# Arash-san/YinYang-Game-AlphaZero

Measured on AMD Instinct MI355X. Metric: self-play positions/sec (+ MCTS node-expansions/sec) at 800 sims, 8x8 board, higher is better.
Workload: dtype f16x3; 1 GPU; 8x8 board, 800 sims/move, 4096 concurrent games per GPU, frozen random-init 128x10 net (seed 0), copied boards, reference_quirks=False, staggered start plies; tree_arithmetic=f32 PUCT + u64 bitboards, nn_dtype=f16x3, evaluation_reuse=False, parallelism=episode-sharded x1, lanes_per_gpu=2, hipgraph=True

## Files before the change

### yinyang-game-alphazero_amd/csrc/yy_common.h

```cpp
#pragma once
#include <hip/hip_runtime.h>
#include <stdio.h>

#include "../../include/yy_engine.h"

extern "C" int yy_tower_set_err(int code, const char *msg);

extern "C" __attribute__((visibility("hidden"))) int yy_mcts_step_noise(yy_mcts *ctx, const float *policy, const float *value, const double *noise, double eps,
                                  float *planes, uint8_t *needs_eval, yy_stream_t stream);

static inline int yy_hip_fail(const char *what, hipError_t e) {
    char msg[512];
    snprintf(msg, sizeof msg, "%s: %s", what, hipGetErrorString(e));
    return yy_tower_set_err(YY_E_HIP, msg);
}
#define HIP_TRY(x)                                        \
    do {                                                  \
        hipError_t e_ = (x);                              \
        if (e_ != hipSuccess) return yy_hip_fail(#x, e_); \
    } while (0)

__device__ __forceinline__ float relu_keep_nan(float v) { return __builtin_isnan(v) ? v : fmaxf(v, 0.0f); }

template <int N> __device__ __forceinline__ void wait_vmcnt() { asm volatile("s_waitcnt vmcnt(%0)" ::"n"(N) : "memory"); }
```

### yinyang-game-alphazero_amd/csrc/yy_engine.hip

```cpp
#include <hip/hip_runtime.h>
#include <math.h>
#include <stdio.h>
#include <string.h>

#include "../../include/yy_engine.h"
#include "yy_bitboard.h"
#include "yy_common.h"
#include "yy_tree.h"

#define YY_VERSION 109

static thread_local char g_err[512] = "";
static int set_err(int code, const char *fmt, const char *a = "", const char *b = "") {
    snprintf(g_err, sizeof g_err, fmt, a, b);
    return code;
}

extern "C" const char *yy_last_error(void) { return g_err; }
extern "C" int yy_tower_set_err(int code, const char *msg) { return set_err(code, "%s%s", msg); }
extern "C" int yy_version(void) { return YY_VERSION; }

static int check_geo(int G, int R, int C) {
    if (G <= 0 || R <= 0 || C <= 0) return set_err(YY_E_INVALID, "non-positive size%s%s");
    if (R > YY_MAX_DIM || C > YY_MAX_DIM || R * C > 64 * YY_MAX_NW)
// ... 624 lines not shown
            const int cell = j * 64 + lane;
            if ((mask.w[j] >> lane) & 1) {
                float p = prow[d.sym ? sym_cell(d.geo, s, cell) : cell];
                bad |= (p != p);
                if (mix) {
                    const float kp = __fmul_rn(keep, p);
                    p = (float)__dadd_rn((double)kp, __dmul_rn(eps, noise[(size_t)g * A + cell]));
                }
                edges[base + mbcnt(mask.w[j])] =
                    make_uint4(__float_as_uint(p), 0u, 0u, CHILD_NONE | ((uint32_t)cell << 24));
            }
            base += yy_popc64(mask.w[j]);
        }
        if (__ballot(bad)) return false;
        if (lane == 0) {
            nodes[node] = make_uint4((uint32_t)n_edges, node_pack(k, (hold && k == 0) ? NF_HASVALUE : 0u, lplayer), 0u,
                                     __float_as_uint(v));
            st->ctr[3] += (uint64_t)k;
        }
        n_edges += k;
    }
    if (lane == 0) {
        st->n_nodes = n_nodes;
        st->n_edges = n_edges;
    }
    return true;
}

__device__ __forceinline__ void backup_path(uint4 *edges, const int32_t *path, const int depth, const float v,
                                            const bool v_is_py, GameState *st) {
    const int lane = lane_id();
    for (int i = lane; i < depth; i += 64) {
        uint4 *e = edges + path[i];
        const int dist = depth - (i + 1);
        const float sv = (dist & 1) ? -v : v;
        uint4 r = *e;
        r.y = (uint32_t)((int)r.y + 1);
        r.z = __float_as_uint(__fadd_rn(__uint_as_float(r.z), sv));
        *e = r;
    }
    if (lane == 0) {
        const float sv = (depth & 1) ? -v : v;
        st->root_N += 1;
        if (st->root_w_is_py && v_is_py && depth == 0) {
            st->root_W_py += (double)((sv == 0.0001f) ? 0.0001 : (sv == -0.0001f ? -0.0001 : (double)sv));
        } else {
            const float base = st->root_w_is_py ? (float)st->root_W_py : st->root_W;
            st->root_W = __fadd_rn(base, sv);
            st->root_w_is_py = 0;
        }
    }
}

template <int NW> __global__ void __launch_bounds__(64) k_begin(MctsDev d, MultiDev m, int target, int kept_target,
                                                                const int32_t *budgets, int max_sims, const int8_t *boards,
                                                                const int8_t *players, const uint8_t *active,
                                                                float *planes) {
    const int g = blockIdx.x;
    const int K = m.K;
    GameState *st = d.state + g;
    LeafRec *rec = K > 1 ? m.leaves + (size_t)g * K : &st->leaf;
    const bool act = active ? (active[g] != 0) : true;
    BB<NW> black, white;
    board_to_bb<NW>(boards + (size_t)g * d.geo.A, d.geo.A, black, white);
    bool keep = false;
    if (rfl((int)st->kept)) {
        const uint64_t *nb = d.nboard + (size_t)g * d.node_cap * 2 * NW;
        const BB<NW> kb = bb_uniform_load<NW>(nb), kw = bb_uniform_load<NW>(nb + NW);
        bool same = act && rfl((int)players[g]) == rfl((int)st->root_player);
#pragma unroll
        for (int i = 0; i < NW; i++) same = same && kb.w[i] == black.w[i] && kw.w[i] == white.w[i];
        keep = same;
    }
    if (keep) {
        if (lane_id() == 0) {
            st->kept = 0;
            st->root_kept = 1;
            st->active = 1;
            st->err = 0;
            st->budget = budgets ? min(max(budgets[g], 0), max_sims) : kept_target;
            rec->kind = K_ROOTKEPT;
            rec->node = 0;
            rec->path_len = 0;
            rec->dup = -1;
        }
    }
    root_setup<NW>(d, st, rec, g, black, white, rfl((int)players[g]), act, keep,
                   budgets ? min(max(budgets[g], 0), max_sims) : target, planes + (size_t)g * K * 5 * d.geo.A);
    if (K > 1 && lane_id() == 0) {
        m.mst[2 * g] = budgets ? min(max(budgets[g], 0), max_sims) : target;
        m.mst[2 * g + 1] = act ? 1 : 0;
    }
}

template <int NW>
__device__ __forceinline__ void do_select(const MctsDev &d, const int g, float *planes, uint8_t *needs_eval,
                                          const uint32_t stamp) {
    GameState *st = d.state + g;
    const int lane = lane_id();
    const int s_active = st->active, s_err = st->err, s_budget = st->budget;
    const int s_kept = st->root_kept;
    int s_carry = st->root_N;
    s_carry = rfl(s_carry);
    if ((rfl(s_active) == 0) | (rfl(s_err) != 0) | (s_carry >= rfl(s_budget))) {
        if (lane == 0) {
            st->leaf.kind = K_NONE;
            if (needs_eval) needs_eval[g] = 0;
        }
        return;
    }
    s_carry -= rfl(s_kept);
// ... 137 lines not shown
    }
    if (!any) return;
    const float keep = (float)(1.0 - eps);
    for (int j = lane; j < k; j += 64) {
        uint4 *e = edges + first + j;
        const float kp = __fmul_rn(keep, __uint_as_float(e->x));
        e->x = __float_as_uint((float)__dadd_rn((double)kp, __dmul_rn(eps, nrow[e->w >> 24])));
    }
}

template <int NW>
__device__ __forceinline__ void do_expand_backup(const MctsDev &d, const int g, const float *policy,
                                                 const float *value, const double *noise, const double eps,
                                                 const uint32_t stamp) {
    GameState *st = d.state + g;
    const int lane = lane_id();
    const int kind = rfl((int)st->leaf.kind);
    if (kind == K_NONE) return;
    const uint4 *nodes = d.nodes + (size_t)g * d.node_cap;
    uint4 *edges = d.edges + (size_t)g * d.edge_cap;
    if (kind == K_ROOTKEPT) {
        if (noise) noise_kept_root(d, g, nodes, edges, noise, eps);
        if (lane == 0) st->leaf.kind = K_NONE;
        return;
    }
    const int32_t *path = d.path + (size_t)g * d.path_cap;
    const int depth = rfl(st->leaf.path_len);
    const int node = rfl(st->leaf.node);
    float v;
    bool v_is_py = false;
    if (kind == K_TERMINAL) {
        v = rflf(__uint_as_float(nodes[node].z));
        v_is_py = true;
    } else if (kind == K_REUSE) {
        v = rflf(__uint_as_float(nodes[node].w));
    } else {
        const bool root = kind == K_ROOTINIT;
        const int src = (root || !(d.ec.meta || d.bk.meta || d.sh.meta)) ? SRC_NONE : rfl(st->leaf_src);
        const LeafEval ev = leaf_eval<NW>(d, g, src, policy, root ? nullptr : value);
        v = ev.v;
        const bool hold = d.reuse && !root;
        if (!expand_leaf<NW>(d, st, g, &st->leaf, path, ev.prow, v, hold, d.aliased != 0u, root ? noise : nullptr, eps)) {
            if (lane == 0) { st->err = st->err_ever = 1; st->leaf.kind = K_NONE; }
            return;
        }
        if (d.ec.meta && src == SRC_NONE && !root) cache_store<NW>(d, st, g, policy, v);
        if (d.sh.meta && src == SRC_NONE && !root) shared_store<NW>(d, st, g, policy, v, stamp);
    }
    if (lane == 0) st->leaf.kind = K_NONE;
    if (kind == K_ROOTINIT) return;
    backup_path(edges, path, depth, v, v_is_py, st);
}

template <int NW> __global__ void __launch_bounds__(64) k_mcts(MctsDev d, int do_backup, int do_sel,
                                                               const float *policy, const float *value,
                                                               const double *noise, double eps, float *planes,
                                                               uint8_t *needs_eval) {
    const int g = blockIdx.x;
    const uint32_t stamp = d.sh.meta ? rfl(*d.sh_stamp) : 0u;
    if (do_backup) do_expand_backup<NW>(d, g, policy, value, noise, eps, stamp);
    if (do_backup && do_sel) __syncthreads();
    if (do_sel) do_select<NW>(d, g, planes, needs_eval, stamp);
}

__global__ void k_stamp(uint32_t *stamp) {
    if (blockIdx.x != 0 || threadIdx.x != 0) return;
    *stamp = sh_next_stamp(*stamp);
}

template <int NW>
__device__ __forceinline__ void do_select_multi(const MctsDev &d, const MultiDev &m, const int g, float *planes,
                                                uint8_t *needs_eval) {
    GameState *st = d.state + g;
    const int lane = lane_id();
    const int K = m.K;
    int32_t *ms = m.mst + 2 * g;
    int keff = 0;
    if (rfl((int)st->active) && !rfl((int)st->err)) keff = min(K, max(0, rfl(ms[0]) - rfl(st->root_N)));
    const GeoBB<NW> gb = geo_bb<NW>(d.geo);
    const uint4 *nodes = d.nodes + (size_t)g * d.node_cap;
    const uint4 *edges = d.edges + (size_t)g * d.edge_cap;
    uint64_t c_levels = 0, c_scan = 0, c_evals = 0, c_term = 0;
    bool failed = false;
    for (int j = 0; j < keff; j++) {
        int32_t *path = d.path + ((size_t)g * K + j) * d.path_cap;
        int node = 0, depth = 0, parent = -1, action = -1, kind;
        uint64_t match = (1ull << j) - 1ull;
        for (;;) {
            const uint4 hdr = nodes[node];
            const uint32_t hy = rfl(hdr.y);
            const int k = node_k(hy), first = rfl((int)hdr.x);
            if (node_flags(hy) & NF_TERMINAL) { kind = K_TERMINAL; break; }
            if (k == 0) { kind = (node == 0) ? K_ROOTPASS : K_REEXPAND; break; }
            if (depth >= (int)d.path_cap) { kind = K_NONE; break; }
            const int vi = ((match >> lane) & 1) ? d.path[((size_t)g * K + lane) * d.path_cap + depth] - first : -1;
            int v[NW];
#pragma unroll
            for (int t = 0; t < NW; t++) v[t] = 0;
            for (uint64_t mm = match; mm; mm &= mm - 1ull) {
                const int c = __builtin_amdgcn_readlane(vi, (int)__ffsll((unsigned long long)mm) - 1);
#pragma unroll
                for (int t = 0; t < NW; t++) v[t] += (c == t * 64 + lane) ? 1 : 0;
            }
            uint4 e[NW];
            uint32_t part = 0;
#pragma unroll
            for (int t = 0; t < NW; t++) {
                const int jj = t * 64 + lane;
                e[t] = (jj < k) ? edges[first + jj] : make_uint4(0u, 0u, 0u, 0u);
                part += e[t].y + (uint32_t)v[t];
            }
            const int S = (int)wave_uadd(part);
            const float sq = d.sqrt_tab[min(S, d.sqrt_n - 1)];
            float q0 = 0.0f;
// ... 7 lines not shown
                    }
                }
                q0 = fpu_value(fp, depth == 0 ? d.fpu_root : d.fpu);
            }
            uint32_t bk = 0, bw = 0;
            int bi = BEST_NONE;
#pragma unroll
            for (int t = 0; t < NW; t++) {
                const int jj = t * 64 + lane;
                if (jj < k) {
                    const float W = __uint_as_float(e[t].z);
                    const float w = (v[t] > 0) ? __fsub_rn(W, (float)v[t]) : W;
                    const uint32_t key = child_key(d.cpuct, sq, __uint_as_float(e[t].x), (int)e[t].y + v[t], w, q0);
                    if (key > bk) { bk = key; bi = jj; bw = e[t].w; }
                }
            }
            const int best = best_child(bk, bi, k);
            if (best == BEST_NONE) { kind = K_NONE; break; }
            const uint32_t w = (uint32_t)__builtin_amdgcn_readlane((int)bw, best & 63);
            if (lane == 0) path[depth] = first + best;
            match = __ballot(vi == best);
            depth++;
            c_levels++;
            c_scan += (uint64_t)k;
            parent = node;
            action = (int)(w >> 24);
            const uint32_t child = w & CHILD_NONE;
            if (child == CHILD_NONE) { kind = K_EXPAND; node = -1; break; }
            node = (int)child;
        }
        if (kind == K_NONE) { failed = true; break; }
        const int dup = match ? (int)__ffsll((unsigned long long)match) - 1 : -1;
        const bool need = (kind == K_EXPAND || kind == K_REEXPAND || kind == K_ROOTPASS) && dup < 0;
        LeafRec *rec = m.leaves + (size_t)g * K + j;
        if (need) {
            BB<NW> black, white;
            const int lplayer = leaf_position<NW>(d, st, g, nodes, kind, parent, action, false, black, white);
            BB<NW> mask;
            bool term;
            float tv;
            leaf_rules<NW>(d.geo, gb, black, white, lplayer, mask, term, tv);
            write_eval_planes<NW>(planes + ((size_t)g * K + j) * 5 * d.geo.A, d.geo, d.sym, d.sym_seed, black, white);
            leaf_store<NW>(rec, black, white, mask, lplayer, term, tv);
        }
        if (lane == 0) {
            rec->kind = (uint8_t)kind;
            rec->node = node;
            rec->path_len = depth;
            rec->dup = dup;
            if (needs_eval) needs_eval[(size_t)g * K + j] = need;
        }
        c_evals += need ? 1 : 0;
        c_term += (kind == K_TERMINAL) ? 1 : 0;
        __syncthreads();
    }
    if (failed && lane == 0) st->err = st->err_ever = 1;
    if (needs_eval && lane < K && (failed || lane >= keff)) needs_eval[(size_t)g * K + lane] = 0;
    if (lane == 0) {
        ms[1] = failed ? 0 : keff;
        st->ctr[1] += c_levels;
        st->ctr[2] += c_scan;
        if (!failed) st->ctr[0] += c_evals;
        st->ctr[4] += c_term;
    }
}

template <int NW>
__device__ __forceinline__ void do_expand_backup_multi(const MctsDev &d, const MultiDev &m, const int g, const float *policy,
                                                       const float *value, const double *noise, const double eps) {
    GameState *st = d.state + g;
    const int lane = lane_id();
    const int K = m.K;
    int32_t *ms = m.mst + 2 * g;
    const int nl = rfl(ms[1]);
    if (nl == 0) return;
    const uint4 *nodes = d.nodes + (size_t)g * d.node_cap;
    uint4 *edges = d.edges + (size_t)g * d.edge_cap;
    for (int j = 0; j < nl; j++) {
        const LeafRec *rec = m.leaves + (size_t)g * K + j;
        const int kind = rfl((int)rec->kind);
        const int depth = rfl(rec->path_len);
        const int dup = rfl(rec->dup);
        const int32_t *path = d.path + ((size_t)g * K + j) * d.path_cap;
        const size_t row = (size_t)g * K + (dup >= 0 ? dup : j);
        float v;
        bool v_is_py = false;
        if (kind == K_TERMINAL) {
            v = rflf(__uint_as_float(nodes[rfl(rec->node)].z));
            v_is_py = true;
        } else if (dup >= 0) {
            v = rflf(value[row]);
        } else {
            v = (kind == K_ROOTINIT) ? 0.0f : rflf(value[row]);
            if (!expand_leaf<NW>(d, st, g, rec, path, policy + row * d.geo.A, v, false, false, noise, eps)) {
                if (lane == 0) { st->err = st->err_ever = 1; ms[1] = 0; }
                return;
            }
        }
        if (kind == K_ROOTINIT) break;
        backup_path(edges, path, depth, v, v_is_py, st);
        __syncthreads();
    }
    if (lane == 0) ms[1] = 0;
}

template <int NW> __global__ void __launch_bounds__(64) k_mcts_multi(MctsDev d, MultiDev m, int do_backup, int do_sel,
                                                                     const float *policy, const float *value,
                                                                     const double *noise, double eps, float *planes,
                                                                     uint8_t *needs_eval) {
    const int g = blockIdx.x;
    if (do_backup) do_expand_backup_multi<NW>(d, m, g, policy, value, noise, eps);
    if (do_backup && do_sel) __syncthreads();
    if (do_sel) do_select_multi<NW>(d, m, g, planes, needs_eval);
}

template <int NW> __global__ void __launch_bounds__(64) k_advance(MctsDev d, const int32_t *actions, int32_t *kept_visits,
                                                                  int32_t *remap_all) {
    __shared__ int32_t win[64];
    const int g = blockIdx.x, lane = lane_id();
    GameState *st = d.state + g;
    uint4 *nodes = d.nodes + (size_t)g * d.node_cap;
    uint4 *edges = d.edges + (size_t)g * d.edge_cap;
    uint64_t *nboard = d.nboard + (size_t)g * d.node_cap * 2 * NW;
    int32_t *remap = remap_all + (size_t)g * d.node_cap;
    const int n_nodes = rfl(st->n_nodes), n_edges = rfl(st->n_edges);
    const int a = rfl(actions[g]);
    const uint4 rhdr = nodes[0];
    const int rk = node_k(rfl(rhdr.y)), rfirst = rfl((int)rhdr.x);
    int child = -1, keptN = 0;
    float keptW = 0.0f;
    bool ok = rfl((int)st->active) != 0 && rfl((int)st->err) == 0 && a >= 0 && a < d.geo.A && n_nodes <= (int)d.node_cap &&
              rk > 0 && rfirst >= 0 && rfirst + rk <= n_edges && n_edges <= (int)d.edge_cap;
    if (ok) {
        ok = false;
        for (int j0 = 0; j0 < rk; j0 += 64) {
            const int j = j0 + lane;
            const uint4 e = (j < rk) ? edges[rfirst + j] : make_uint4(0u, 0u, 0u, 0xFF000000u | CHILD_NONE);
            const uint64_t hit = __ballot(j < rk && (int)(e.w >> 24) == a);
            if (hit) {
                const int l = (int)__ffsll((unsigned long long)hit) - 1;
                const uint32_t w = (uint32_t)__builtin_amdgcn_readlane((int)e.w, l);
                keptN = __builtin_amdgcn_readlane((int)e.y, l);
                keptW = __uint_as_float((uint32_t)__builtin_amdgcn_readlane((int)e.z, l));
                child = (int)(w & CHILD_NONE);
                ok = (w & CHILD_NONE) != CHILD_NONE && child > 0 && child < n_nodes;
                break;
            }
        }
    }
    uint32_t chy = 0;
    if (ok) {
        chy = rfl(nodes[child].y);
        ok = !(node_flags(chy) & NF_TERMINAL) && node_k(chy) > 0;
    }
    if (!ok) {
        if (lane == 0) {
            st->kept = 0;
            st->n_nodes = 1;
            st->n_edges = 0;
            st->root_N = 0;
            st->root_W = 0.0f;
            st->root_W_py = 0.0;
            st->root_w_is_py = 1;
            nodes[0] = make_uint4(0u, node_pack(0, 0, node_player(rfl(rhdr.y))), 0u, 0u);
            if (kept_visits) kept_visits[g] = 0;
// ... 20 lines not shown
            for (int j0 = 0; j0 < k; j0 += 64) {
                const int j = j0 + lane;
                if (j < k) {
                    const uint4 e = edges[first + j];
                    edges[ne + j] = e;
                    const int c = (int)(e.w & CHILD_NONE);
                    if ((e.w & CHILD_NONE) != CHILD_NONE && c > i && c < n_nodes) {
                        if (c < base + 64) win[c - base] = 0;
                        else remap[c] = 0;
                    }
                }
            }
            if (lane == 0) {
                nodes[rank] = make_uint4(k > 0 ? (uint32_t)ne : 0u, hy, (uint32_t)__builtin_amdgcn_readlane((int)hdr.z, t),
                                         (uint32_t)__builtin_amdgcn_readlane((int)hdr.w, t));
                remap[i] = rank;
            }
            if (rank != i && lane < 2 * NW) nboard[(size_t)rank * 2 * NW + lane] = nboard[(size_t)i * 2 * NW + lane];
            rank++;
            ne += k;
            __syncthreads();
        }
        if (bad) break;
    }
    __syncthreads();
    if (!bad)
        for (int e = lane; e < ne; e += 64) {
            const uint32_t w = edges[e].w;
            const uint32_t c = w & CHILD_NONE;
            if (c != CHILD_NONE) {
                const int nc = (c < (uint32_t)n_nodes) ? remap[c] : -1;
                edges[e].w = (w & 0xFF000000u) | (nc >= 0 ? (uint32_t)nc : CHILD_NONE);
            }
        }
    if (lane == 0) {
        if (bad) {
            st->err = st->err_ever = 1;
            st->kept = 0;
            if (kept_visits) kept_visits[g] = 0;
        } else {
            st->n_nodes = rank;
            st->n_edges = ne;
            st->root_N = keptN;
            st->root_W = keptW;
            st->root_W_py = 0.0;
            st->root_w_is_py = 0;
            st->root_player = (int8_t)node_player(chy);
            st->kept = 1;
            if (kept_visits) kept_visits[g] = keptN;
        }
    }
}

template <int NW> __global__ void __launch_bounds__(64) k_root_counts(MctsDev d, int32_t *counts, float *cw, float *cp) {
    const int g = blockIdx.x, A = d.geo.A;
    const uint4 hdr = d.nodes[(size_t)g * d.node_cap];
    const int k = node_k(rfl(hdr.y)), first = rfl((int)hdr.x);
    const bool act = rfl((int)d.state[g].active) != 0;
    for (int a = lane_id(); a < A; a += 64) {
        counts[(size_t)g * A + a] = 0;
        if (cw) cw[(size_t)g * A + a] = 0.0f;
        if (cp) cp[(size_t)g * A + a] = 0.0f;
    }
    __syncthreads();
    if (!act) return;
    const uint4 *edges = d.edges + (size_t)g * d.edge_cap;
    for (int j = lane_id(); j < k; j += 64) {
        const uint4 e = edges[first + j];
        const int a = (int)(e.w >> 24);
        counts[(size_t)g * A + a] = (int)e.y;
        if (cw) cw[(size_t)g * A + a] = __uint_as_float(e.z);
        if (cp) cp[(size_t)g * A + a] = __uint_as_float(e.x);
    }
}

template <int NW> __global__ void __launch_bounds__(64) k_root_policy(MctsDev d, int tzero, double *pi) {
    root_distribution<NW>(d, blockIdx.x, tzero, pi + (size_t)blockIdx.x * d.geo.A);
}

__global__ void k_root_stats(MctsDev d, int32_t *visits, double *wsum) {
    const int g = blockIdx.x * blockDim.x + threadIdx.x;
    if (g >= d.G) return;
    const GameState *st = d.state + g;
    if (visits) visits[g] = st->root_N;
    if (wsum) wsum[g] = st->root_w_is_py ? st->root_W_py : (double)st->root_W;
}

template <int NW> __global__ void __launch_bounds__(64) k_get_boards(MctsDev d, int8_t *boards) {
    const int g = blockIdx.x;
    const uint64_t *src = d.gboard + (size_t)g * 2 * NW;
    BB<NW> b = bb_uniform_load<NW>(src), w = bb_uniform_load<NW>(src + NW);
    bb_to_board<NW>(boards + (size_t)g * d.geo.A, d.geo.A, b, w);
}

__global__ void k_status(MctsDev d, uint64_t *out ) {
    uint64_t acc[9] = {0, 0, 0, 0, 0, 0, 0, 0, 0};
    for (int g = blockIdx.x * blockDim.x + threadIdx.x; g < d.G; g += gridDim.x * blockDim.x) {
        GameState *st = d.state + g;
        for (int i = 0; i < 8; i++) acc[i] += st->ctr[i];
        acc[8] += (st->err || st->err_ever) ? 1 : 0;
        st->err_ever = 0;
    }
    for (int i = 0; i < 9; i++)
        if (acc[i]) atomicAdd((unsigned long long *)&out[i], (unsigned long long)acc[i]);
}

__global__ void k_reset_counters(MctsDev d) {
    const int g = blockIdx.x * blockDim.x + threadIdx.x;
    if (g >= d.G) return;
    for (int i = 0; i < 8; i++) d.state[g].ctr[i] = 0;
    d.state[g].forced = 0;
    for (int i = 0; i < 4; i++) d.state[g].shc[i] = 0;
    if (g == 0 && d.sh_sweep) d.sh_sweep[SH_SW_EVICTED] = 0;
}

__global__ void k_forced_sum(MctsDev d, uint64_t *out) {
    uint64_t acc = 0;
    for (int g = blockIdx.x * blockDim.x + threadIdx.x; g < d.G; g += gridDim.x * blockDim.x) acc += d.state[g].forced;
    if (acc) atomicAdd((unsigned long long *)out, (unsigned long long)acc);
}

extern "C" int yy_mcts_create(const yy_mcts_config *cfg, yy_mcts **out) {
    if (!cfg || !out) return set_err(YY_E_INVALID, "null pointer%s%s");
    if (int e = check_geo(cfg->G, cfg->R, cfg->C)) return e;
    if (cfg->max_sims < 1) return set_err(YY_E_INVALID, "max_sims < 1%s%s");
    if ((cfg->flags & YY_FLAG_REUSE_PASS_VALUE) && (cfg->flags & YY_FLAG_ALIASED))
        return set_err(YY_E_INVALID, "YY_FLAG_REUSE_PASS_VALUE needs copied boards: with the aliased board a node's position changes between visits%s%s");
    if ((cfg->flags & YY_FLAG_EVAL_SYMMETRY) && (cfg->flags & YY_FLAG_ALIASED))
        return set_err(YY_E_UNSUPPORTED, "YY_FLAG_EVAL_SYMMETRY needs copied boards (YY_FLAG_ALIASED reproduces the reference, which has no such option)%s%s");
    if (cfg->flags & YY_FLAG_FORCED_PLAYOUTS) {
// ... 76 lines not shown
            *a.p = nullptr;
            yy_mcts_destroy(c);
            return set_err(YY_E_NOMEM, "hipMalloc failed: %s%s", hipGetErrorString(me), what);
        }
        c->bytes += a.n;
    }
    float *tab = new float[d.sqrt_n];
    for (int s = 0; s < d.sqrt_n; s++) tab[s] = (float)sqrt((double)s);
    hipError_t e = hipMemset(d.state, 0, G * sizeof(GameState));
    if (e == hipSuccess) e = hipMemset(d.nodes, 0, G * d.node_cap * sizeof(uint4));
    if (e == hipSuccess && d.ec.meta) e = hipMemset(d.ec.meta, 0, G * (size_t)ec_cap * sizeof(uint32_t));
    if (e == hipSuccess && m.mst) e = hipMemset(m.mst, 0, G * 2 * sizeof(int32_t));
    if (e == hipSuccess) e = hipMemcpy(d.sqrt_tab, tab, (size_t)d.sqrt_n * sizeof(float), hipMemcpyHostToDevice);
    if (e == hipSuccess) e = hipDeviceSynchronize();
    delete[] tab;
    if (e != hipSuccess) { yy_mcts_destroy(c); return set_err(YY_E_HIP, "arena initialisation: %s%s", hipGetErrorString(e)); }
    *out = c;
    return YY_OK;
}

extern "C" int yy_mcts_destroy(yy_mcts *c) {
    if (!c) return YY_OK;
    const MctsDev &d = c->dev;
    void *ps[] = {d.edges, d.nodes, d.nboard, d.gboard, d.path, d.state, d.sqrt_tab, c->scratch, d.ec.meta, d.ec.key, d.ec.val, d.ec.pol,
                  c->multi.leaves, c->multi.mst, c->remap};
    for (void *p : ps)
        if (p) (void)hipFree(p);
    delete c;
    return YY_OK;
}

extern "C" int yy_mcts_set_num_sims(yy_mcts *c, int32_t num_sims) {
    if (!c) return set_err(YY_E_INVALID, "null pointer%s%s");
    if (num_sims < 0 || num_sims > c->cfg.max_sims) return set_err(YY_E_INVALID, "num_sims outside 0 .. max_sims%s%s");
    c->target_sims = num_sims == 0 ? c->cfg.max_sims : num_sims;
    return YY_OK;
}

extern "C" int yy_mcts_set_sim_budgets(yy_mcts *c, const int32_t *budgets_dev) {
    if (!c) return set_err(YY_E_INVALID, "null pointer%s%s");
    c->budgets = budgets_dev;
    return YY_OK;
}

extern "C" int yy_mcts_memory_bytes(const yy_mcts *c, uint64_t *out) {
    if (!c || !out) return set_err(YY_E_INVALID, "null pointer%s%s");
    *out = c->bytes;
    return YY_OK;
}

extern "C" int yy_mcts_begin(yy_mcts *c, const int8_t *boards, const int8_t *players, const uint8_t *active,
                             float *planes, yy_stream_t s) {
    if (!c || !boards || !players || !planes) return set_err(YY_E_INVALID, "null pointer%s%s");
    DISPATCH_NW(c->dev.geo.NW, k_begin<NW><<<dim3(c->cfg.G), dim3(64), 0, (hipStream_t)s>>>(c->dev, c->multi,
                                                   c->multi.K > 1 ? c->target_sims : 0x7FFFFFFF, c->target_sims, c->budgets, c->cfg.max_sims,
                                                   boards, players, active, planes));
    HIP_TRY(hipGetLastError());
    c->pending = 2;
    return YY_OK;
}

extern "C" int yy_mcts_advance(yy_mcts *c, const int32_t *actions, int32_t *kept_visits, yy_stream_t s) {
    if (!c || !actions) return set_err(YY_E_INVALID, "null pointer%s%s");
    if (c->cfg.flags & YY_FLAG_ALIASED)
        return set_err(YY_E_UNSUPPORTED, "yy_mcts_advance needs copied boards: with the aliased board a node's position changes between visits%s%s");
    if (c->multi.K > 1) return set_err(YY_E_UNSUPPORTED, "yy_mcts_advance: leaves_per_step > 1 does not support tree reuse%s%s");
    if (c->pending != 0) return set_err(YY_E_STATE, "yy_mcts_advance with a select or a root expansion pending%s%s");
    if (!c->remap) {
        const size_t n = (size_t)c->cfg.G * c->dev.node_cap * sizeof(int32_t);
        const hipError_t me = hipMalloc((void **)&c->remap, n);
        if (me != hipSuccess) {
            (void)hipGetLastError();
            c->remap = nullptr;
            return set_err(YY_E_NOMEM, "hipMalloc failed: %s%s", hipGetErrorString(me), " (tree reuse remap array)");
        }
        c->bytes += n;
    }
    DISPATCH_NW(c->dev.geo.NW, k_advance<NW><<<dim3(c->cfg.G), dim3(64), 0, (hipStream_t)s>>>(c->dev, actions, kept_visits, c->remap));
    HIP_TRY(hipGetLastError());
    return YY_OK;
}

static int launch_mcts(yy_mcts *c, int backup, int sel, const float *policy, const float *value, const double *noise,
                       double eps, float *planes, uint8_t *needs_eval, yy_stream_t s) {
    if (c->dev.sh.meta) {
        hipLaunchKernelGGL(k_stamp, dim3(1), dim3(1), 0, (hipStream_t)s, c->dev.sh_stamp);
        HIP_TRY(hipGetLastError());
    }
    if (c->multi.K > 1) {
        DISPATCH_NW(c->dev.geo.NW, k_mcts_multi<NW><<<dim3(c->cfg.G), dim3(64), 0, (hipStream_t)s>>>(c->dev, c->multi, backup, sel,
                                                       policy, value, noise, eps, planes, needs_eval));
    } else {
        DISPATCH_NW(c->dev.geo.NW, k_mcts<NW><<<dim3(c->cfg.G), dim3(64), 0, (hipStream_t)s>>>(c->dev, backup, sel,
                                                       policy, value, noise, eps, planes, needs_eval));
    }
    HIP_TRY(hipGetLastError());
    return YY_OK;
}

extern "C" int yy_mcts_expand_root(yy_mcts *c, const float *policy, const double *noise, double eps, yy_stream_t s) {
    if (!c || !policy) return set_err(YY_E_INVALID, "null pointer%s%s");
    if (c->pending != 2) return set_err(YY_E_STATE, "yy_mcts_expand_root without yy_mcts_begin%s%s");
    int e = launch_mcts(c, 1, 0, policy, nullptr, noise, eps, nullptr, nullptr, s);
    if (e == YY_OK) c->pending = 0;
    return e;
}

extern "C" int yy_mcts_select(yy_mcts *c, float *planes, uint8_t *needs_eval, yy_stream_t s) {
    if (!c || !planes) return set_err(YY_E_INVALID, "null pointer%s%s");
    if (c->pending != 0) return set_err(YY_E_STATE, "yy_mcts_select with an expansion pending%s%s");
    int e = launch_mcts(c, 0, 1, nullptr, nullptr, nullptr, 0.0, planes, needs_eval, s);
    if (e == YY_OK) c->pending = 1;
    return e;
}

extern "C" int yy_mcts_expand_backup(yy_mcts *c, const float *policy, const float *value, yy_stream_t s) {
    if (!c || !policy || !value) return set_err(YY_E_INVALID, "null pointer%s%s");
    if (c->pending != 1) return set_err(YY_E_STATE, "yy_mcts_expand_backup without yy_mcts_select%s%s");
    int e = launch_mcts(c, 1, 0, policy, value, nullptr, 0.0, nullptr, nullptr, s);
    if (e == YY_OK) c->pending = 0;
    return e;
}

extern "C" int yy_mcts_step(yy_mcts *c, const float *policy, const float *value, float *planes, uint8_t *needs_eval,
                            yy_stream_t s) {
    if (!c || !policy || !value || !planes) return set_err(YY_E_INVALID, "null pointer%s%s");
    if (c->pending != 1) return set_err(YY_E_STATE, "yy_mcts_step without a pending select%s%s");
    return launch_mcts(c, 1, 1, policy, value, nullptr, 0.0, planes, needs_eval, s);
}

extern "C" __attribute__((visibility("hidden"))) int yy_mcts_step_noise(yy_mcts *c, const float *policy, const float *value, const double *noise, double eps,
                                  float *planes, uint8_t *needs_eval, yy_stream_t s) {
    return launch_mcts(c, 1, 1, policy, value, noise, eps, planes, needs_eval, s);
}

extern "C" int yy_mcts_root_counts(yy_mcts *c, int32_t *counts, float *cw, float *cp, yy_stream_t s) {
    if (!c || !counts) return set_err(YY_E_INVALID, "null pointer%s%s");
    DISPATCH_NW(c->dev.geo.NW,
                k_root_counts<NW><<<dim3(c->cfg.G), dim3(64), 0, (hipStream_t)s>>>(c->dev, counts, cw, cp));
    HIP_TRY(hipGetLastError());
    return YY_OK;
}

extern "C" int yy_mcts_root_policy(yy_mcts *c, int tzero, double *pi, yy_stream_t s) {
    if (!c || !pi) return set_err(YY_E_INVALID, "null pointer%s%s");
    DISPATCH_NW(c->dev.geo.NW,
                k_root_policy<NW><<<dim3(c->cfg.G), dim3(64), 0, (hipStream_t)s>>>(c->dev, tzero, pi));
    HIP_TRY(hipGetLastError());
    return YY_OK;
}

extern "C" int yy_mcts_root_stats(yy_mcts *c, int32_t *visits, double *wsum, yy_stream_t s) {
    if (!c) return set_err(YY_E_INVALID, "null pointer%s%s");
    hipLaunchKernelGGL(k_root_stats, dim3((c->cfg.G + 255) / 256), dim3(256), 0, (hipStream_t)s, c->dev, visits, wsum);
    HIP_TRY(hipGetLastError());
    return YY_OK;
}

extern "C" int yy_mcts_get_boards(yy_mcts *c, int8_t *boards, yy_stream_t s) {
    if (!c || !boards) return set_err(YY_E_INVALID, "null pointer%s%s");
    DISPATCH_NW(c->dev.geo.NW, k_get_boards<NW><<<dim3(c->cfg.G), dim3(64), 0, (hipStream_t)s>>>(c->dev, boards));
    HIP_TRY(hipGetLastError());
    return YY_OK;
}

extern "C" int yy_mcts_status(yy_mcts *c, int32_t *n_overflow, uint64_t *counters) {
    if (!c) return set_err(YY_E_INVALID, "null pointer%s%s");
    HIP_TRY(hipDeviceSynchronize());
    HIP_TRY(hipMemset(c->scratch, 0, 9 * sizeof(uint64_t)));
    hipLaunchKernelGGL(k_status, dim3(64), dim3(256), 0, 0, c->dev, c->scratch);
    HIP_TRY(hipGetLastError());
    uint64_t h[9];
    HIP_TRY(hipMemcpy(h, c->scratch, sizeof h, hipMemcpyDeviceToHost));
    if (counters) {
        for (int i = 0; i < 8; i++) counters[i] = h[i];
    }
    if (n_overflow) *n_overflow = (int32_t)h[8];
    if (h[8]) return set_err(YY_E_ARENA, "tree arena overflow or non-finite evaluator output in at least one game since the last status call%s%s");
    return YY_OK;
}

extern "C" int yy_mcts_forced_descents(yy_mcts *c, uint64_t *out) {
    if (!c || !out) return set_err(YY_E_INVALID, "null pointer%s%s");
    HIP_TRY(hipDeviceSynchronize());
    HIP_TRY(hipMemset(c->scratch, 0, sizeof(uint64_t)));
    hipLaunchKernelGGL(k_forced_sum, dim3(64), dim3(256), 0, 0, c->dev, c->scratch);
    HIP_TRY(hipGetLastError());
    HIP_TRY(hipMemcpy(out, c->scratch, sizeof(uint64_t), hipMemcpyDeviceToHost));
    return YY_OK;
}

template <int NW> __global__ void k_book_insert(const uint64_t *__restrict__ keys, int n, uint32_t *meta, uint64_t *tkeys,
                                                uint32_t mask, int32_t *slot_of) {
    const int i = blockIdx.x * blockDim.x + threadIdx.x;
    if (i >= n) return;
    const uint64_t *k = keys + (size_t)i * 2 * NW;
    const int got = tt_probe(bb_hash<NW>(k, k + NW), mask,
                             [&](uint32_t at) { return atomicCAS(&meta[at], 0u, 1u) == 0u ? TT_HIT : TT_NEXT; });
    if (got >= 0)
        for (int j = 0; j < 2 * NW; j++) tkeys[(size_t)got * 2 * NW + j] = k[j];
// ... 130 lines not shown
```

### yinyang-game-alphazero_amd/csrc/yy_nn_epilogue.hip

```cpp
#include <hip/hip_runtime.h>
#include <math.h>
#include <stdint.h>

#include "../../include/yy_engine.h"
#include "yy_common.h"

typedef __attribute__((ext_vector_type(8))) unsigned short us8;

__device__ __forceinline__ float bf2f(unsigned short h) { return __uint_as_float(((uint32_t)h) << 16); }
__device__ __forceinline__ unsigned short f2bf(float f) {
    uint32_t u = __float_as_uint(f);
    if ((u & 0x7FFFFFFFu) > 0x7F800000u) return (unsigned short)((u >> 16) | 0x40u);
    return (unsigned short)((u + 0x7FFFu + ((u >> 16) & 1u)) >> 16);
}

template <bool HAS_RES, bool RELU, bool FIXED>
__global__ void __launch_bounds__(256) k_bias_act(us8 *x, const float *bias, const us8 *res, size_t n_vec, int cvec) {
    const size_t tid = (size_t)blockIdx.x * blockDim.x + threadIdx.x;
    const size_t stride = (size_t)gridDim.x * blockDim.x;
    float b[8];
    if (FIXED) {
        const float4 *bp = reinterpret_cast<const float4 *>(bias + (tid % (size_t)cvec) * 8);
        const float4 b0 = bp[0], b1 = bp[1];
        b[0] = b0.x; b[1] = b0.y; b[2] = b0.z; b[3] = b0.w;
// ... 19 lines not shown
        x[i] = o;
    }
}

template <bool FIXED>
static void launch_bias_act(us8 *xv, const float *bias, const us8 *rv, size_t n_vec, int cvec, int relu, unsigned blocks,
                            hipStream_t st) {
    if (rv) {
        if (relu) k_bias_act<true, true, FIXED><<<dim3(blocks), dim3(256), 0, st>>>(xv, bias, rv, n_vec, cvec);
        else k_bias_act<true, false, FIXED><<<dim3(blocks), dim3(256), 0, st>>>(xv, bias, rv, n_vec, cvec);
    } else {
        if (relu) k_bias_act<false, true, FIXED><<<dim3(blocks), dim3(256), 0, st>>>(xv, bias, rv, n_vec, cvec);
        else k_bias_act<false, false, FIXED><<<dim3(blocks), dim3(256), 0, st>>>(xv, bias, rv, n_vec, cvec);
    }
}

extern "C" int yy_nn_bias_act_bf16(void *x, const float *bias, const void *residual, int64_t rows, int C, int relu,
                                   yy_stream_t s) {
    if (rows == 0) return YY_OK;
    if (!x || !bias || rows < 0 || C <= 0) return yy_tower_set_err(YY_E_INVALID, "bad argument");
    if (C % 8) return yy_tower_set_err(YY_E_UNSUPPORTED, "channels must be a multiple of 8");
    const int cvec = C / 8;
    const size_t n_vec = (size_t)rows * (size_t)cvec;
    size_t blocks = (n_vec + 255) / 256;
    if (blocks > 256 * 8) blocks = 256 * 8;
    const bool fixed = (256 % cvec) == 0;
    if (fixed) launch_bias_act<true>((us8 *)x, bias, (const us8 *)residual, n_vec, cvec, relu, (unsigned)blocks, (hipStream_t)s);
    else launch_bias_act<false>((us8 *)x, bias, (const us8 *)residual, n_vec, cvec, relu, (unsigned)blocks, (hipStream_t)s);
    HIP_TRY(hipGetLastError());
    return YY_OK;
}

__global__ void __launch_bounds__(64) k_head_finish(const unsigned short *__restrict__ h, int A, int H,
                                                    const float *__restrict__ w2, const float *__restrict__ b2,
                                                    float *__restrict__ policy, float *__restrict__ value) {
    const int g = blockIdx.x, lane = threadIdx.x;
    const unsigned short *row = h + (size_t)g * (A + H);
    float mx = -INFINITY;
    for (int a = lane; a < A; a += 64) mx = fmaxf(mx, bf2f(row[a]));
#pragma unroll
    for (int o = 32; o > 0; o >>= 1) mx = fmaxf(mx, __shfl_xor(mx, o, 64));
    float sum = 0.0f;
    for (int a = lane; a < A; a += 64) sum += expf(bf2f(row[a]) - mx);
#pragma unroll
    for (int o = 32; o > 0; o >>= 1) sum += __shfl_xor(sum, o, 64);
    for (int a = lane; a < A; a += 64) policy[(size_t)g * A + a] = expf(bf2f(row[a]) - mx) / sum;
    float acc = 0.0f;
    for (int j = lane; j < H; j += 64) acc += fmaxf(bf2f(row[A + j]), 0.0f) * w2[j];
#pragma unroll
    for (int o = 32; o > 0; o >>= 1) acc += __shfl_xor(acc, o, 64);
    if (lane == 0) value[g] = tanhf(acc + b2[0]);
}

__global__ void __launch_bounds__(64) k_head_finish_f32(const float *__restrict__ logits, const float *__restrict__ hidden,
                                                        int A, int H, const float *__restrict__ w2,
                                                        const float *__restrict__ b2, const int32_t *__restrict__ rows,
                                                        const int32_t *__restrict__ n_rows, float *__restrict__ policy,
                                                        float *__restrict__ value) {
    const int i = blockIdx.x, lane = threadIdx.x;
    if (n_rows && i >= *n_rows) return;
    const int g = rows ? rows[i] : i;
    const float *row = logits + (size_t)i * A;
    float mx = -INFINITY;
    for (int a = lane; a < A; a += 64) mx = fmaxf(mx, row[a]);
#pragma unroll
    for (int o = 32; o > 0; o >>= 1) mx = fmaxf(mx, __shfl_xor(mx, o, 64));
    float sum = 0.0f;
    for (int a = lane; a < A; a += 64) sum += expf(row[a] - mx);
#pragma unroll
    for (int o = 32; o > 0; o >>= 1) sum += __shfl_xor(sum, o, 64);
    for (int a = lane; a < A; a += 64) policy[(size_t)g * A + a] = expf(row[a] - mx) / sum;
    const float *hr = hidden + (size_t)i * H;
    float acc = 0.0f;
    for (int j = lane; j < H; j += 64) acc += relu_keep_nan(hr[j]) * w2[j];
#pragma unroll
    for (int o = 32; o > 0; o >>= 1) acc += __shfl_xor(acc, o, 64);
    if (lane == 0) value[g] = tanhf(acc + b2[0]);
}

extern "C" int yy_nn_head_finish_f32(const float *logits, const float *hidden, int G, int A, int H, const float *w2,
                                     const float *b2, const int32_t *rows, const int32_t *n_rows, float *policy, float *value,
                                     yy_stream_t s) {
    if (G == 0) return YY_OK;
    if (!logits || !hidden || !w2 || !b2 || !policy || !value || G < 0 || A <= 0 || H <= 0 || (rows && !n_rows))
        return yy_tower_set_err(YY_E_INVALID, "bad argument");
    k_head_finish_f32<<<dim3(G), dim3(64), 0, (hipStream_t)s>>>(logits, hidden, A, H, w2, b2, rows, n_rows, policy, value);
    HIP_TRY(hipGetLastError());
    return YY_OK;
}

__global__ void __launch_bounds__(1024) k_compact_rows(const uint8_t *__restrict__ flags, int G, int32_t *__restrict__ rows,
                                                       int32_t *__restrict__ n) {
    __shared__ int wsum[16];
    const int t = threadIdx.x, lane = t & 63, wave = t >> 6;
    const int per = (G + 1023) / 1024, lo = min(t * per, G), hi = min(lo + per, G);
    int cnt = 0;
    for (int g = lo; g < hi; g++) cnt += flags[g] != 0;
    int incl = cnt;
#pragma unroll
    for (int o = 1; o < 64; o <<= 1) {
        const int v = __shfl_up(incl, o, 64);
        if (lane >= o) incl += v;
    }
    if (lane == 63) wsum[wave] = incl;
    __syncthreads();
    int base = 0;
    for (int w = 0; w < wave; w++) base += wsum[w];
    int pos = base + incl - cnt;
    for (int g = lo; g < hi; g++)
        if (flags[g] != 0) rows[pos++] = g;
    if (t == 1023) *n = base + incl;
}

extern "C" int yy_compact_rows(const uint8_t *flags, int G, int32_t *rows, int32_t *n, yy_stream_t s) {
    if (!flags || !rows || !n || G < 0) return yy_tower_set_err(YY_E_INVALID, "bad argument");
    k_compact_rows<<<dim3(1), dim3(1024), 0, (hipStream_t)s>>>(flags, G, rows, n);
    HIP_TRY(hipGetLastError());
    return YY_OK;
}

extern "C" int yy_nn_head_finish_bf16(const void *h, int G, int A, int H, const float *w2, const float *b2, float *policy,
                                      float *value, yy_stream_t s) {
    if (G == 0) return YY_OK;
    if (!h || !w2 || !b2 || !policy || !value || G < 0 || A <= 0 || H <= 0) return yy_tower_set_err(YY_E_INVALID, "bad argument");
    k_head_finish<<<dim3(G), dim3(64), 0, (hipStream_t)s>>>((const unsigned short *)h, A, H, w2, b2, policy, value);
    HIP_TRY(hipGetLastError());
    return YY_OK;
}
```

### yinyang-game-alphazero_amd/csrc/yy_tree.h

```cpp
#pragma once
#include <hip/hip_runtime.h>
#include <stdint.h>

#include "../../include/yy_engine.h"
#include "yy_bitboard.h"
#include "yy_draws.h"

__device__ __forceinline__ uint32_t rfl(uint32_t v) { return __builtin_amdgcn_readfirstlane(v); }
__device__ __forceinline__ int rfl(int v) { return (int)__builtin_amdgcn_readfirstlane((uint32_t)v); }
__device__ __forceinline__ uint64_t rfl64(uint64_t v) {
    return ((uint64_t)rfl((uint32_t)(v >> 32)) << 32) | rfl((uint32_t)v);
}
__device__ __forceinline__ float rflf(float v) { return __uint_as_float(rfl(__float_as_uint(v))); }
__device__ __forceinline__ int lane_id() { return threadIdx.x & 63; }
__device__ __forceinline__ int mbcnt(uint64_t m) {
    return __builtin_amdgcn_mbcnt_hi((uint32_t)(m >> 32), __builtin_amdgcn_mbcnt_lo((uint32_t)m, 0));
}
__device__ __forceinline__ int wave_sum(int v) {
#pragma unroll
    for (int o = 32; o > 0; o >>= 1) v += __shfl_xor(v, o, 64);
    return v;
}

template <int NW> __device__ __forceinline__ BB<NW> bb_uniform_load(const uint64_t *p) {
    BB<NW> r;
#pragma unroll
    for (int i = 0; i < NW; i++) r.w[i] = rfl64(p[i]);
    return r;
}
template <int NW> __device__ __forceinline__ void bb_store_lane0(uint64_t *p, BB<NW> b) {
    if (lane_id() == 0) {
#pragma unroll
        for (int i = 0; i < NW; i++) p[i] = b.w[i];
    }
}

template <int NW>
__device__ __forceinline__ void board_to_bb(const int8_t *b, int A, BB<NW> &black, BB<NW> &white) {
#pragma unroll
    for (int j = 0; j < NW; j++) {
        int cell = j * 64 + lane_id();
        int v = (cell < A) ? (int)b[cell] : 0;
        black.w[j] = __ballot(v == 1);
        white.w[j] = __ballot(v == -1);
    }
}
template <int NW>
__device__ __forceinline__ void bb_to_board(int8_t *b, int A, BB<NW> black, BB<NW> white) {
#pragma unroll
    for (int j = 0; j < NW; j++) {
        int cell = j * 64 + lane_id();
        if (cell < A)
            b[cell] = ((black.w[j] >> lane_id()) & 1) ? 1 : (((white.w[j] >> lane_id()) & 1) ? -1 : 0);
    }
}

template <int NW> __device__ __forceinline__ uint32_t bb_row_bits(BB<NW> occ, int r, int C) {
    int s = r * C, w = s >> 6, o = s & 63;
// ... 342 lines not shown
        const uint4 e = edges[first + j];
        const float P = __uint_as_float(e.x), w = __uint_as_float(e.z);
        const int n = cn[i];
        const double bound = forced_bound(d.forced, P, S);
        int np = n;
        for (int m = 0; np >= 1 && __dmul_rn((double)m, (double)m) < bound; m++) {
            if (child_key_at(d.cpuct, sq, P, np - 1, n, w) < kstar) np -= 1;
            else break;
        }
        cn[i] = (np == 1) ? 0 : np;
    }
}

template <int NW> __device__ __forceinline__ void root_distribution(const MctsDev &d, const int g, const int tzero, double *pi) {
    const int A = d.geo.A;
    const uint4 hdr = d.nodes[(size_t)g * d.node_cap];
    const int k = node_k(rfl(hdr.y)), first = rfl((int)hdr.x);
    const uint4 *edges = d.edges + (size_t)g * d.edge_cap;
    const bool act = rfl((int)d.state[g].active) != 0;
    int cn[NW];
    int sum = 0, mx = 0;
#pragma unroll
    for (int i = 0; i < NW; i++) {
        const int j = i * 64 + lane_id();
        cn[i] = (act && j < k) ? (int)edges[first + j].y : 0;
        sum += cn[i];
    }
    sum = wave_sum(sum);
    if (d.forced > 0.0 && act) {
        prune_forced<NW>(d, edges, first, k, sum, cn);
        sum = 0;
#pragma unroll
        for (int i = 0; i < NW; i++) sum += cn[i];
        sum = wave_sum(sum);
    }
#pragma unroll
    for (int i = 0; i < NW; i++) mx = max(mx, cn[i]);
#pragma unroll
    for (int o = 32; o > 0; o >>= 1) mx = max(mx, __shfl_xor(mx, o, 64));
    double fill;
    int nbest = 0;
    if (tzero) {
        if (mx == 0) nbest = A;
        else {
#pragma unroll
            for (int i = 0; i < NW; i++) nbest += (i * 64 + lane_id() < k && cn[i] == mx);
            nbest = wave_sum(nbest);
        }
        fill = (mx == 0) ? 1.0 / (double)A : 0.0;
    } else {
        fill = (sum > 0) ? 0.0 : 1.0 / (double)A;
    }
    for (int a = lane_id(); a < A; a += 64) pi[a] = act ? fill : 0.0;
    __syncthreads();
    if (!act) return;
    if (tzero ? (mx > 0) : (sum > 0)) {
#pragma unroll
        for (int i = 0; i < NW; i++) {
            const int j = i * 64 + lane_id();
            if (j < k) {
                const int a = (int)(edges[first + j].w >> 24), n = cn[i];
                pi[a] = tzero ? ((n == mx) ? 1.0 / (double)nbest : 0.0) : (double)n / (double)sum;
            }
        }
    }
}
```

Measured before the change: 1826 positions/s.

## Pack multiple games per workgroup, one wavefront each, with wave-level syncs

Game-parallel kernels (begin, mcts, mcts_multi, root counts/policy, head finish) now launch workgroups of up to 16 wavefronts, one game per wave, instead of one 64-thread block per game. Block-wide __syncthreads are replaced by wave-scoped fences plus a wave barrier, which also lets early-returning waves exit safely. The aim is to cut workgroup dispatch overhead and raise occupancy for 4096 games. The cost is that any code relying on block-wide shared memory or LDS would now be shared across waves, and the launch bounds may constrain register allocation.

```diff
diff --git a/yinyang-game-alphazero_amd/csrc/yy_common.h b/yinyang-game-alphazero_amd/csrc/yy_common.h
--- a/yinyang-game-alphazero_amd/csrc/yy_common.h
+++ b/yinyang-game-alphazero_amd/csrc/yy_common.h
@@ -22,4 +22,21 @@
 
 __device__ __forceinline__ float relu_keep_nan(float v) { return __builtin_isnan(v) ? v : fmaxf(v, 0.0f); }
 
+#ifndef YY_WPB
+#define YY_WPB 16
+#endif
+static_assert(YY_WPB >= 1 && YY_WPB <= 16, "a workgroup has at most 16 wavefronts");
+#define YY_WAVE_ITEM_BOUNDS __launch_bounds__(64 * YY_WPB, (2 * YY_WPB + 3) / 4)
+static inline dim3 games_grid(int G) { return dim3((unsigned)((G + YY_WPB - 1) / YY_WPB)); }
+static inline dim3 games_block() { return dim3(64 * YY_WPB); }
+__device__ __forceinline__ int game_of_wave(int n) {
+    const int g = __builtin_amdgcn_readfirstlane((int)(blockIdx.x * YY_WPB + (threadIdx.x >> 6)));
+    return g < n ? g : -1;
+}
+__device__ __forceinline__ void wave_sync() {
+    __builtin_amdgcn_fence(__ATOMIC_RELEASE, "workgroup");
+    __builtin_amdgcn_wave_barrier();
+    __builtin_amdgcn_fence(__ATOMIC_ACQUIRE, "workgroup");
+}
+
 template <int N> __device__ __forceinline__ void wait_vmcnt() { asm volatile("s_waitcnt vmcnt(%0)" ::"n"(N) : "memory"); }
diff --git a/yinyang-game-alphazero_amd/csrc/yy_engine.hip b/yinyang-game-alphazero_amd/csrc/yy_engine.hip
--- a/yinyang-game-alphazero_amd/csrc/yy_engine.hip
+++ b/yinyang-game-alphazero_amd/csrc/yy_engine.hip
@@ -700,11 +700,12 @@
     }
 }
 
-template <int NW> __global__ void __launch_bounds__(64) k_begin(MctsDev d, MultiDev m, int target, int kept_target,
+template <int NW> __global__ void YY_WAVE_ITEM_BOUNDS k_begin(MctsDev d, MultiDev m, int target, int kept_target,
                                                                 const int32_t *budgets, int max_sims, const int8_t *boards,
                                                                 const int8_t *players, const uint8_t *active,
                                                                 float *planes) {
-    const int g = blockIdx.x;
+    const int g = game_of_wave(d.G);
+    if (g < 0) return;
     const int K = m.K;
     GameState *st = d.state + g;
     LeafRec *rec = K > 1 ? m.leaves + (size_t)g * K : &st->leaf;
@@ -948,14 +949,15 @@
     backup_path(edges, path, depth, v, v_is_py, st);
 }
 
-template <int NW> __global__ void __launch_bounds__(64) k_mcts(MctsDev d, int do_backup, int do_sel,
+template <int NW> __global__ void YY_WAVE_ITEM_BOUNDS k_mcts(MctsDev d, int do_backup, int do_sel,
                                                                const float *policy, const float *value,
                                                                const double *noise, double eps, float *planes,
                                                                uint8_t *needs_eval) {
-    const int g = blockIdx.x;
+    const int g = game_of_wave(d.G);
+    if (g < 0) return;
     const uint32_t stamp = d.sh.meta ? rfl(*d.sh_stamp) : 0u;
     if (do_backup) do_expand_backup<NW>(d, g, policy, value, noise, eps, stamp);
-    if (do_backup && do_sel) __syncthreads();
+    if (do_backup && do_sel) wave_sync();
     if (do_sel) do_select<NW>(d, g, planes, needs_eval, stamp);
 }
 
@@ -1069,7 +1071,7 @@
         }
         c_evals += need ? 1 : 0;
         c_term += (kind == K_TERMINAL) ? 1 : 0;
-        __syncthreads();
+        wave_sync();
     }
     if (failed && lane == 0) st->err = st->err_ever = 1;
     if (needs_eval && lane < K && (failed || lane >= keff)) needs_eval[(size_t)g * K + lane] = 0;
@@ -1116,18 +1118,19 @@
         }
         if (kind == K_ROOTINIT) break;
         backup_path(edges, path, depth, v, v_is_py, st);
-        __syncthreads();
+        wave_sync();
     }
     if (lane == 0) ms[1] = 0;
 }
 
-template <int NW> __global__ void __launch_bounds__(64) k_mcts_multi(MctsDev d, MultiDev m, int do_backup, int do_sel,
+template <int NW> __global__ void YY_WAVE_ITEM_BOUNDS k_mcts_multi(MctsDev d, MultiDev m, int do_backup, int do_sel,
                                                                      const float *policy, const float *value,
                                                                      const double *noise, double eps, float *planes,
                                                                      uint8_t *needs_eval) {
-    const int g = blockIdx.x;
+    const int g = game_of_wave(d.G);
+    if (g < 0) return;
     if (do_backup) do_expand_backup_multi<NW>(d, m, g, policy, value, noise, eps);
-    if (do_backup && do_sel) __syncthreads();
+    if (do_backup && do_sel) wave_sync();
     if (do_sel) do_select_multi<NW>(d, m, g, planes, needs_eval);
 }
 
@@ -1254,8 +1257,9 @@
     }
 }
 
-template <int NW> __global__ void __launch_bounds__(64) k_root_counts(MctsDev d, int32_t *counts, float *cw, float *cp) {
-    const int g = blockIdx.x, A = d.geo.A;
+template <int NW> __global__ void YY_WAVE_ITEM_BOUNDS k_root_counts(MctsDev d, int32_t *counts, float *cw, float *cp) {
+    const int g = game_of_wave(d.G), A = d.geo.A;
+    if (g < 0) return;
     const uint4 hdr = d.nodes[(size_t)g * d.node_cap];
     const int k = node_k(rfl(hdr.y)), first = rfl((int)hdr.x);
     const bool act = rfl((int)d.state[g].active) != 0;
@@ -1264,7 +1268,7 @@
         if (cw) cw[(size_t)g * A + a] = 0.0f;
         if (cp) cp[(size_t)g * A + a] = 0.0f;
     }
-    __syncthreads();
+    wave_sync();
     if (!act) return;
     const uint4 *edges = d.edges + (size_t)g * d.edge_cap;
     for (int j = lane_id(); j < k; j += 64) {
@@ -1276,8 +1280,10 @@
     }
 }
 
-template <int NW> __global__ void __launch_bounds__(64) k_root_policy(MctsDev d, int tzero, double *pi) {
-    root_distribution<NW>(d, blockIdx.x, tzero, pi + (size_t)blockIdx.x * d.geo.A);
+template <int NW> __global__ void YY_WAVE_ITEM_BOUNDS k_root_policy(MctsDev d, int tzero, double *pi) {
+    const int g = game_of_wave(d.G);
+    if (g < 0) return;
+    root_distribution<NW>(d, g, tzero, pi + (size_t)g * d.geo.A);
 }
 
 __global__ void k_root_stats(MctsDev d, int32_t *visits, double *wsum) {
@@ -1460,7 +1466,7 @@
 extern "C" int yy_mcts_begin(yy_mcts *c, const int8_t *boards, const int8_t *players, const uint8_t *active,
                              float *planes, yy_stream_t s) {
     if (!c || !boards || !players || !planes) return set_err(YY_E_INVALID, "null pointer%s%s");
-    DISPATCH_NW(c->dev.geo.NW, k_begin<NW><<<dim3(c->cfg.G), dim3(64), 0, (hipStream_t)s>>>(c->dev, c->multi,
+    DISPATCH_NW(c->dev.geo.NW, k_begin<NW><<<games_grid(c->cfg.G), games_block(), 0, (hipStream_t)s>>>(c->dev, c->multi,
                                                    c->multi.K > 1 ? c->target_sims : 0x7FFFFFFF, c->target_sims, c->budgets, c->cfg.max_sims,
                                                    boards, players, active, planes));
     HIP_TRY(hipGetLastError());
@@ -1496,10 +1502,10 @@
         HIP_TRY(hipGetLastError());
     }
     if (c->multi.K > 1) {
-        DISPATCH_NW(c->dev.geo.NW, k_mcts_multi<NW><<<dim3(c->cfg.G), dim3(64), 0, (hipStream_t)s>>>(c->dev, c->multi, backup, sel,
+        DISPATCH_NW(c->dev.geo.NW, k_mcts_multi<NW><<<games_grid(c->cfg.G), games_block(), 0, (hipStream_t)s>>>(c->dev, c->multi, backup, sel,
                                                        policy, value, noise, eps, planes, needs_eval));
     } else {
-        DISPATCH_NW(c->dev.geo.NW, k_mcts<NW><<<dim3(c->cfg.G), dim3(64), 0, (hipStream_t)s>>>(c->dev, backup, sel,
+        DISPATCH_NW(c->dev.geo.NW, k_mcts<NW><<<games_grid(c->cfg.G), games_block(), 0, (hipStream_t)s>>>(c->dev, backup, sel,
                                                        policy, value, noise, eps, planes, needs_eval));
     }
     HIP_TRY(hipGetLastError());
@@ -1545,7 +1551,7 @@
 extern "C" int yy_mcts_root_counts(yy_mcts *c, int32_t *counts, float *cw, float *cp, yy_stream_t s) {
     if (!c || !counts) return set_err(YY_E_INVALID, "null pointer%s%s");
     DISPATCH_NW(c->dev.geo.NW,
-                k_root_counts<NW><<<dim3(c->cfg.G), dim3(64), 0, (hipStream_t)s>>>(c->dev, counts, cw, cp));
+                k_root_counts<NW><<<games_grid(c->cfg.G), games_block(), 0, (hipStream_t)s>>>(c->dev, counts, cw, cp));
     HIP_TRY(hipGetLastError());
     return YY_OK;
 }
@@ -1553,7 +1559,7 @@
 extern "C" int yy_mcts_root_policy(yy_mcts *c, int tzero, double *pi, yy_stream_t s) {
     if (!c || !pi) return set_err(YY_E_INVALID, "null pointer%s%s");
     DISPATCH_NW(c->dev.geo.NW,
-                k_root_policy<NW><<<dim3(c->cfg.G), dim3(64), 0, (hipStream_t)s>>>(c->dev, tzero, pi));
+                k_root_policy<NW><<<games_grid(c->cfg.G), games_block(), 0, (hipStream_t)s>>>(c->dev, tzero, pi));
     HIP_TRY(hipGetLastError());
     return YY_OK;
 }
diff --git a/yinyang-game-alphazero_amd/csrc/yy_nn_epilogue.hip b/yinyang-game-alphazero_amd/csrc/yy_nn_epilogue.hip
--- a/yinyang-game-alphazero_amd/csrc/yy_nn_epilogue.hip
+++ b/yinyang-game-alphazero_amd/csrc/yy_nn_epilogue.hip
@@ -95,13 +95,13 @@
     if (lane == 0) value[g] = tanhf(acc + b2[0]);
 }
 
-__global__ void __launch_bounds__(64) k_head_finish_f32(const float *__restrict__ logits, const float *__restrict__ hidden,
-                                                        int A, int H, const float *__restrict__ w2,
+__global__ void YY_WAVE_ITEM_BOUNDS k_head_finish_f32(const float *__restrict__ logits, const float *__restrict__ hidden,
+                                                        int G, int A, int H, const float *__restrict__ w2,
                                                         const float *__restrict__ b2, const int32_t *__restrict__ rows,
                                                         const int32_t *__restrict__ n_rows, float *__restrict__ policy,
                                                         float *__restrict__ value) {
-    const int i = blockIdx.x, lane = threadIdx.x;
-    if (n_rows && i >= *n_rows) return;
+    const int i = game_of_wave(G), lane = threadIdx.x & 63;
+    if (i < 0 || (n_rows && i >= *n_rows)) return;
     const int g = rows ? rows[i] : i;
     const float *row = logits + (size_t)i * A;
     float mx = -INFINITY;
@@ -127,7 +127,7 @@
     if (G == 0) return YY_OK;
     if (!logits || !hidden || !w2 || !b2 || !policy || !value || G < 0 || A <= 0 || H <= 0 || (rows && !n_rows))
         return yy_tower_set_err(YY_E_INVALID, "bad argument");
-    k_head_finish_f32<<<dim3(G), dim3(64), 0, (hipStream_t)s>>>(logits, hidden, A, H, w2, b2, rows, n_rows, policy, value);
+    k_head_finish_f32<<<games_grid(G), games_block(), 0, (hipStream_t)s>>>(logits, hidden, G, A, H, w2, b2, rows, n_rows, policy, value);
     HIP_TRY(hipGetLastError());
     return YY_OK;
 }
diff --git a/yinyang-game-alphazero_amd/csrc/yy_tree.h b/yinyang-game-alphazero_amd/csrc/yy_tree.h
--- a/yinyang-game-alphazero_amd/csrc/yy_tree.h
+++ b/yinyang-game-alphazero_amd/csrc/yy_tree.h
@@ -4,6 +4,7 @@
 
 #include "../../include/yy_engine.h"
 #include "yy_bitboard.h"
+#include "yy_common.h"
 #include "yy_draws.h"
 
 __device__ __forceinline__ uint32_t rfl(uint32_t v) { return __builtin_amdgcn_readfirstlane(v); }
@@ -452,7 +453,7 @@
         fill = (sum > 0) ? 0.0 : 1.0 / (double)A;
     }
     for (int a = lane_id(); a < A; a += 64) pi[a] = act ? fill : 0.0;
-    __syncthreads();
+    wave_sync();
     if (!act) return;
     if (tzero ? (mx > 0) : (sum > 0)) {
 #pragma unroll
```

Result: no change. 1823 positions/s (-0.1%).
